# HpWang-whu/RoReg

Hardware: AMD Instinct MI355X
Metric: pair-registrations/sec (higher is better)
Workload: dtype f32 (every f32 operand enters the fp16 matrix cores as hi + lo fp16 under a per-keypoint power-of-two block scale: <= 22 significant bits relative to a CONSERVATIVE per-keypoint bound -- measured on the extractor: the bound sits 2^2..2^6 above the keypoint's true coefficient maximum (config.f16x2_sc

## Files before the change

include/roreg_hip.h:

```cpp
#ifndef ROREG_HIP_H
#define ROREG_HIP_H

#include <stdint.h>
#include <stddef.h>

#ifdef __cplusplus
extern "C" {
#endif

#define ROREG_ABI_VERSION 6
int roreg_abi_version(void);
const char *roreg_last_error(void);

int roreg_set_group_tables(const int32_t *P_host, const int32_t *Nei_host, const double *R_host);

size_t roreg_group_conv_packed_size(int Cin, int Cout, int KS);
int roreg_group_conv_pack_weights(const float *W_host , int Cin, int Cout, int KS,
                                  float *wpack_host );
size_t roreg_group_conv_workspace_size(int B, int Cin, int Cout, int Lin, int Lout, int KS);
int roreg_group_conv(const float *x, const float *wpack, const float *bias,
                     const float *bn_scale, const float *bn_shift, const float *residual,
                     float *out, const int32_t *gather,
                     int B, int Cin, int Cout, int Lin, int Lout, int KS,
                     float *workspace, size_t workspace_floats, void *stream);
// ... 175 lines not shown

int roreg_knn_attention(const float *qp, const float *kp, const float *vp, const int64_t *idx, int k_is_table, int v_is_table,
                        int m, int k, float *x_out, void *stream);

int roreg_rm_elementwise(int op, const float *a, const float *b, const float *c, const int64_t *idx, int L, int k, int C,
                         float *out, float *ws, void *stream);

size_t roreg_sinkhorn_workspace_size(int m, int n);
int roreg_sinkhorn(const float *src_final, int m, const float *tgt_final, int n, float alpha, int iters, float *Z_out,
                   int64_t *matches0, int64_t *matches1, float *mscores0, float *mscores1, float *ws, size_t ws_floats, void *stream);

size_t roreg_sinkhorn_batch_workspace_size(int n_seg, int max_m, int max_n, long long total_m, long long total_n);
int roreg_sinkhorn_batch_consts(const int32_t *seg_src_host, const int32_t *seg_tgt_host, int n_seg, float *consts_host);
int roreg_sinkhorn_batch(const float *src_final, const float *tgt_final, const int32_t *seg_src, const int32_t *seg_tgt,
                         const int32_t *seg_src_host, const int32_t *seg_tgt_host, const float *consts, int n_seg, float alpha, int iters,
                         int64_t *matches0, int64_t *matches1, float *mscores0, float *mscores1, float *ws, size_t ws_floats,
                         void *stream);

size_t roreg_sinkhorn_batch2_workspace_size(int n_seg, int max_m, int max_n, long long total_m, long long total_n);
int roreg_sinkhorn_batch2(const float *src_final, const float *tgt_final, const int32_t *seg_src, const int32_t *seg_tgt,
                          const int32_t *seg_src_host, const int32_t *seg_tgt_host, const float *consts, int n_seg, float alpha, int iters,
                          int64_t *matches0, int64_t *matches1, float *mscores0, float *mscores1, float *ws, size_t ws_floats,
                          int recompute, void *stream);
size_t roreg_sinkhorn_batch3_workspace_size(int n_seg, int max_m, int max_n, long long total_m, long long total_n, int recompute, int want_Z);
int roreg_sinkhorn_batch3(const float *src_final, const float *tgt_final, const int32_t *seg_src, const int32_t *seg_tgt,
                          const int32_t *seg_src_host, const int32_t *seg_tgt_host, const float *consts, int n_seg, float alpha, int iters,
                          int64_t *matches0, int64_t *matches1, float *mscores0, float *mscores1, float *ws, size_t ws_floats,
                          int recompute, float *Z_out, void *stream);
int roreg_write_files(const char *const *paths, const void *const *headers, const int32_t *header_len, const void *const *data,
                      const int64_t *nbytes, int n, int n_threads);
int roreg_yohoc_draw_many(const uint32_t *seeds, int n_pairs, const int64_t *anchors, const int64_t *offsets, int max_iter, int max_tries,
                          int64_t *rows_out, int32_t *n_hyp_out, double *giveup_out, int n_threads);
size_t roreg_mlp_head_workspace(int L, int n_seg, int C1);
int roreg_mlp_head(const float *x, const float *pos, const float *table, const int64_t *idx, const float *conf, int m, int k, int L, int Cin,
                   const float *W1, const float *b1, int C1, const float *Wr, const float *br, float *h, float *y, const int32_t *seg_off,
                   int n_seg, int mult, float eps, float *mean_rstd, double *ws, void *stream);
int roreg_sinkhorn_early_exit(int on);
int roreg_sinkhorn_iteration_stats(long long *iterations, long long *pairs, int reset, void *stream);

int roreg_set_fourier_tables(const float *F_host);
size_t roreg_irrep_gemm_tiles(int O, int B, int32_t *tiles_host);
size_t roreg_irrep_gemm_tiles_m(int O, int B, int tile_m , int32_t *tiles_host);
int roreg_irrep_gemm(const float *const *X, float *const *Out, const float *const *Add, const float *const *Wpack, int C, int O, int B,
                     const int32_t *tiles_dev, int n_tiles, void *stream);
int roreg_irrep_gemm_split(const float *const *X, float *const *Out, const float *const *Add, const void *const *Wsplit, int C, int O, int B,
                           const int32_t *tiles_dev, int n_tiles, void *stream);
int roreg_irrep_gemm_f16x2(const float *const *X, float *const *Out, const float *const *Add, const void *const *Wsplit2,
                           const float *x_bound_dev, int w_exp, const float *next_u_dev, const float *next_v_dev, float *out_bound_dev,
                           int C, int O, int B, const int32_t *tiles_dev, int n_tiles,
                           int tile_m ,
                           int x_planes , void *stream);
int roreg_gemm_persistent(int on);
int roreg_gemm_thin(int on);
int roreg_row_bound(const void *x_spatial, int x_bf16 , const float *bn_scale, const float *bn_shift,
                    float *bound_out, int B, int C, void *stream);
int roreg_ft_nonlin(const float *Xin , const float *x_spatial, const float *bias,
                    const float *bias2, const float *bn_scale, const float *bn_shift, const float *resid_spatial,
                    float *Xout , float *out_spatial ,
                    const int32_t *g_map ,
                    int Lout , int Lvalid,
                    int B, int C, int split ,
                    const float *out_bound ,
                    float *out_rowmax ,
                    int spatial_bf16 ,
                    int out_planes ,
                    void *stream);
int roreg_ft_nonlin_packed(const float *Xin, const float *bias, const float *bn_scale, const float *bn_shift, uint32_t *out_words,
                           const int32_t *g_map, int Lout, int Lvalid, int B, int C, const float *out_bound, float *raw_col, int raw_g,
                           void *stream);
int roreg_ft_nonlin_gathered(const uint64_t *rows , const int64_t *dr , int feat_bf16, const float *bn_scale ,
                             const float *bn_shift, float *Xout, int B, const float *out_bound , int out_planes, void *stream);

typedef struct roreg_icp_grid_desc {
    double origin[3];
    double edge;
    int32_t dims[3];
    int32_t n;
    int64_t cells;
    int64_t reserved;
} roreg_icp_grid_desc;
size_t roreg_icp_grid_size(const double *lo_host, const double *hi_host, int n, double max_dist, roreg_icp_grid_desc *desc_host,
                           size_t *workspace_bytes);
int roreg_icp_grid_build(const float *points, const roreg_icp_grid_desc *desc_host, void *grid, void *workspace, size_t workspace_bytes,
                         void *stream);
typedef struct roreg_icp_task {
    const void *tgt_grid;
    const void *src_grid;
    const double *T0;
    int32_t n_src;
    int32_t slot0;
} roreg_icp_task;
size_t roreg_icp_batch_workspace(int n_tasks, long long total_slots);
int roreg_icp_batch(const roreg_icp_task *tasks, int n_tasks, const int32_t *work, int n_work, long long total_slots, double max_dist,
                    int max_iter, double tol_deg, double tol_t, double *T_out, int32_t *iters_out, int32_t *inliers_out, double *rmse_out,
                    int32_t *status_out, int32_t *assign_out, double *stats_out, void *workspace, size_t workspace_bytes, void *stream);

int roreg_icp_normals(const void *grid, double radius, int min_neighbors, double *out, void *stream);
typedef struct roreg_icp_plane_task {
    const void *tgt_grid;
    const void *src_grid;
    const double *tgt_normals;
    const double *T0;
    int32_t n_src;
    int32_t slot0;
} roreg_icp_plane_task;
size_t roreg_icp_plane_batch_workspace(int n_tasks, long long total_slots);
// ... 49 lines not shown
```

roreg_amd/_abi.py:

```python
import ctypes
from ctypes import c_int, c_void_p, c_size_t, c_double, c_float, c_char_p

import numpy as np

ABI_VERSION = 6

_P = c_void_p
PROTOTYPES = {
    'roreg_abi_version': (c_int, []),
    'roreg_last_error': (c_char_p, []),
    'roreg_set_group_tables': (c_int, [_P, _P, _P]),
    'roreg_group_conv_packed_size': (c_size_t, [c_int, c_int, c_int]),
    'roreg_group_conv_pack_weights': (c_int, [_P, c_int, c_int, c_int, _P]),
    'roreg_group_conv_workspace_size': (c_size_t, [c_int, c_int, c_int, c_int, c_int, c_int]),
    'roreg_group_conv': (c_int, [_P, _P, _P, _P, _P, _P, _P, _P, c_int, c_int, c_int, c_int, c_int, c_int, _P, c_size_t, _P]),
    'roreg_group_conv_split': (c_int, [_P, _P, _P, _P, _P, _P, _P, _P, c_int, c_int, c_int, c_int, c_int, c_int, c_int, _P]),
    'roreg_group_conv_f16x2': (c_int, [_P, _P, c_int, _P, _P, _P, c_float, c_float, _P, _P, _P, _P, _P, c_int, c_int, c_int, c_int, c_int, c_int, c_int, _P]),
    'roreg_group_conv_f16x2_packed': (c_int, [_P, _P, c_int, _P, _P, _P, _P, _P, _P, c_int, c_int, c_int, c_int, c_int, c_int, c_int, _P]),
    'roreg_dense_f16x2': (c_int, [_P, _P, c_int, _P, _P, _P, c_float, c_float, _P, _P, c_int, _P, _P, c_int, c_int, c_int, _P]),
    'roreg_dense_split': (c_int, [_P, _P, _P, _P, _P, _P, c_int, _P, c_int, c_int, c_int, _P]),
    'roreg_gf_finalize': (c_int, [_P, _P, c_int, _P, c_int, _P]),
    'roreg_det_score': (c_int, [_P, _P, c_int, _P]),
    'roreg_inv_descriptor': (c_int, [_P, c_int, _P, c_int, _P]),
    'roreg_nn_search': (c_int, [_P, _P, c_int, _P, _P, c_int, c_int, _P, _P, _P, _P]),
# ... 3 lines not shown
    'roreg_knn_search': (c_int, [_P, c_int, _P, c_int, c_int, c_int, _P, _P, c_size_t, _P]),
    'roreg_knn_search_ex': (c_int, [_P, c_int, _P, c_int, c_int, c_int, c_int, _P, _P, _P, c_size_t, _P]),
    'roreg_knn_search_seg_workspace': (c_size_t, [ctypes.c_longlong, c_int, c_int, c_int]),
    'roreg_knn_search_seg': (c_int, [_P, _P, _P, _P, c_int, ctypes.c_longlong, c_int, c_int, c_int, c_int, _P, _P, c_size_t, _P]),
    'roreg_mutual_matches': (c_int, [_P, _P, c_int, c_int, _P, _P, _P, _P, _P]),
    'roreg_mutual_match_batch_workspace': (c_size_t, [c_int, c_int]),
    'roreg_mutual_match_batch': (c_int, [_P, c_int, c_int, _P, _P, _P, c_size_t, _P]),
    'roreg_des2r': (c_int, [_P, _P, _P, _P, c_int, _P, _P, _P]),
    'roreg_set_des2r_tables': (c_int, [c_int, _P, _P, _P, _P]),
    'roreg_group_corr_irrep': (c_int, [_P, _P, _P, _P, c_int, c_int, _P, _P]),
    'roreg_group_corr_mfma': (c_int, [_P, _P, _P, _P, c_int, c_int, _P, _P]),
    'roreg_des2r_irrep': (c_int, [_P, _P, _P, _P, _P, _P, c_int, c_int, _P, _P]),
    'roreg_des2r_recheck_count': (c_int, [c_int, _P]),
    'roreg_feat_coefs': (c_int, [_P, c_int, _P, c_int, c_int, c_int, _P]),
    'roreg_et_gather': (c_int, [_P, _P, _P, _P, c_int, _P, _P, _P, c_int, _P, _P]),
    'roreg_quat_to_trans': (c_int, [_P, _P, _P, _P, _P, _P, c_int, _P, _P, _P]),
    'roreg_ransac_score': (c_int, [_P, _P, _P, c_int, c_int, _P, _P, c_int, c_double, _P, _P, _P, _P]),
    'roreg_refine': (c_int, [_P, _P, _P, c_int, c_int, _P, c_int, _P, _P, _P, c_double, _P, _P, _P]),
    'roreg_lt_prepare_batch': (c_int, [_P, c_int, c_int, c_int, _P, _P, _P, _P, _P, _P]),
    'roreg_lt_finish_batch': (c_int, [_P, c_int, c_int, _P, _P, _P, _P]),
    'roreg_role_max': (c_int, [_P, _P, c_int, _P, _P, _P, c_int, _P]),
    'roreg_row_bound_roles': (c_int, [_P, c_int, _P, _P, _P, _P, c_int, _P]),
    'roreg_inv_descriptor_roles': (c_int, [_P, c_int, _P, _P, _P, _P, c_int, _P]),
    'roreg_lt_prepare_rows': (c_int, [_P, _P, c_int, c_int, c_int, _P, _P, _P, _P]),
    'roreg_ransac_batch_workspace': (c_size_t, [c_int, ctypes.c_longlong, c_int]),
    'roreg_ransac_batch': (c_int, [_P, c_int, ctypes.c_longlong, c_int, c_int, c_double, c_int, _P, _P, _P, _P, _P, _P, c_size_t, _P]),
    'roreg_refine_batch': (c_int, [_P, _P, c_int, ctypes.c_longlong, _P, ctypes.c_double, c_int, _P, _P, _P, _P]),
    'roreg_yohoc_draw': (c_int, [_P, ctypes.c_longlong, _P, _P, c_int, c_int, _P, _P, _P, _P]),
    'roreg_gather_rows_batch': (c_int, [_P, c_int, c_int, c_int, _P]),
    'roreg_gather_rows_f64': (c_int, [_P, _P, c_int, c_int, _P, _P]),
    'roreg_group_corr': (c_int, [_P, _P, _P, _P, c_int, c_int, _P, _P, _P]),
    'roreg_topk_dot_workspace_size': (c_size_t, [c_int, c_int, c_int]),
    'roreg_topk_dot': (c_int, [_P, c_int, _P, c_int, c_int, _P, _P, _P, c_size_t, _P, _P, c_int, c_int, c_int, _P]),
    'roreg_context_colmax': (c_int, [_P, c_int, _P, c_int, c_int, _P, _P, _P]),
    'roreg_sinkhorn_batch_workspace_size': (c_size_t, [c_int, c_int, c_int, ctypes.c_longlong, ctypes.c_longlong]),
    'roreg_sinkhorn_batch_consts': (c_int, [_P, _P, c_int, _P]),
    'roreg_sinkhorn_batch': (c_int, [_P, _P, _P, _P, _P, _P, _P, c_int, c_float, c_int, _P, _P, _P, _P, _P, c_size_t, _P]),
    'roreg_sinkhorn_batch2_workspace_size': (c_size_t, [c_int, c_int, c_int, ctypes.c_longlong, ctypes.c_longlong]),
    'roreg_sinkhorn_batch2': (c_int, [_P, _P, _P, _P, _P, _P, _P, c_int, c_float, c_int, _P, _P, _P, _P, _P, c_size_t, c_int, _P]),
    'roreg_sinkhorn_batch3_workspace_size': (c_size_t, [c_int, c_int, c_int, ctypes.c_longlong, ctypes.c_longlong, c_int, c_int]),
    'roreg_sinkhorn_batch3': (c_int, [_P, _P, _P, _P, _P, _P, _P, c_int, c_float, c_int, _P, _P, _P, _P, _P, c_size_t, c_int, _P, _P]),
    'roreg_write_files': (c_int, [_P, _P, _P, _P, _P, c_int, c_int]),
    'roreg_yohoc_draw_many': (c_int, [_P, c_int, _P, _P, c_int, c_int, _P, _P, _P, c_int]),
    'roreg_mlp_head_workspace': (c_size_t, [c_int, c_int, c_int]),
    'roreg_mlp_head': (c_int, [_P, _P, _P, _P, _P, c_int, c_int, c_int, c_int, _P, _P, c_int, _P, _P, _P, _P, _P, c_int, c_int, c_float, _P, _P, _P]),
    'roreg_sinkhorn_early_exit': (c_int, [c_int]),
    'roreg_sinkhorn_iteration_stats': (c_int, [_P, _P, c_int, _P]),
    'roreg_linear': (c_int, [_P, c_int, c_int, _P, _P, c_int, _P, _P]),
    'roreg_linear_mfma': (c_int, [_P, c_int, c_int, _P, _P, c_int, _P, _P]),
    'roreg_linear_path': (c_int, [c_int]),
    'roreg_linear_cat3': (c_int, [_P, _P, _P, _P, c_int, c_int, _P, _P, c_int, _P, _P]),
    'roreg_gemm_persistent': (c_int, [c_int]),
    'roreg_gemm_thin': (c_int, [c_int]),
    'roreg_instnorm_stats': (c_int, [_P, c_int, c_int, c_float, _P, _P, _P, c_int, c_int, _P]),
    'roreg_mlp_tail': (c_int, [_P, c_int, c_int, _P, _P, _P, _P, _P, c_int, c_int, _P]),
    'roreg_mlp_tail_mfma': (c_int, [_P, c_int, c_int, _P, _P, _P, _P, _P, c_int, c_int, _P]),
    'roreg_knn_attention': (c_int, [_P, _P, _P, _P, c_int, c_int, c_int, c_int, _P, _P]),
    'roreg_rm_elementwise': (c_int, [c_int, _P, _P, _P, _P, c_int, c_int, c_int, _P, _P, _P]),
    'roreg_sinkhorn_workspace_size': (c_size_t, [c_int, c_int]),
    'roreg_sinkhorn': (c_int, [_P, c_int, _P, c_int, c_float, c_int, _P, _P, _P, _P, _P, _P, c_size_t, _P]),
    'roreg_icp_grid_size': (c_size_t, [_P, _P, c_int, c_double, _P, _P]),
    'roreg_icp_grid_build': (c_int, [_P, _P, _P, _P, c_size_t, _P]),
    'roreg_icp_batch_workspace': (c_size_t, [c_int, ctypes.c_longlong]),
    'roreg_icp_batch': (c_int, [_P, c_int, _P, c_int, ctypes.c_longlong, c_double, c_int, c_double, c_double, _P, _P, _P, _P, _P, _P, _P, _P, c_size_t, _P]),
    'roreg_icp_normals': (c_int, [_P, c_double, c_int, _P, _P]),
    'roreg_icp_plane_batch_workspace': (c_size_t, [c_int, ctypes.c_longlong]),
    'roreg_icp_plane_batch': (c_int, [_P, c_int, _P, c_int, ctypes.c_longlong, c_double, c_int, c_double, c_double, _P, _P, _P, _P, _P, _P, _P, _P, c_size_t, _P]),
    'roreg_icp_gicp_batch_workspace': (c_size_t, [c_int, ctypes.c_longlong]),
    'roreg_icp_gicp_batch': (c_int, [_P, c_int, _P, c_int, ctypes.c_longlong, c_double, c_int, c_double, c_double, _P, _P, _P, _P, _P, _P, _P, _P, c_size_t, _P]),
    'roreg_icp_eval_workspace': (c_size_t, [c_int, ctypes.c_longlong]),
    'roreg_icp_eval_batch': (c_int, [_P, c_int, _P, c_int, ctypes.c_longlong, c_double, _P, _P, _P, _P, _P, c_size_t, _P]),
    'roreg_voxel_workspace': (c_size_t, [c_int]),
    'roreg_voxel_downsample': (c_int, [_P, c_int, c_double, _P, _P, _P, _P, _P, _P, _P, c_size_t, _P]),
    'roreg_pg_workspace': (c_size_t, [_P, c_int]),
    'roreg_pg_optimize_batch': (c_int, [_P, _P, c_int, _P, _P, _P, _P, _P, _P, _P, _P, _P, _P, _P, c_int, c_int, _P, _P, _P, _P, _P, _P, _P, _P, _P, _P, _P, c_size_t, _P]),
    'roreg_profile_enable': (c_int, [c_int]),
    'roreg_profile_read': (c_int, [c_int, _P, _P]),
    'roreg_set_fourier_tables': (c_int, [_P]),
    'roreg_mt_shuffle_prefix': (c_int, [_P, c_int, _P, c_int, c_int, _P, c_int]),
    'roreg_mt_stream_shuffle_prefix': (c_int, [_P, _P, _P, c_int, c_int, _P]),
    'roreg_irrep_gemm_tiles': (c_size_t, [c_int, c_int, _P]),
    'roreg_irrep_gemm_tiles_m': (c_size_t, [c_int, c_int, c_int, _P]),
    'roreg_irrep_gemm': (c_int, [_P, _P, _P, _P, c_int, c_int, c_int, _P, c_int, _P]),
    'roreg_irrep_gemm_split': (c_int, [_P, _P, _P, _P, c_int, c_int, c_int, _P, c_int, _P]),
    'roreg_irrep_gemm_f16x2': (c_int, [_P, _P, _P, _P, _P, c_int, _P, _P, _P, c_int, c_int, c_int, _P, c_int, c_int, c_int, _P]),
    'roreg_row_bound': (c_int, [_P, c_int, _P, _P, _P, c_int, c_int, _P]),
    'roreg_ft_nonlin': (c_int, [_P, _P, _P, _P, _P, _P, _P, _P, _P, _P, c_int, c_int, c_int, c_int, c_int, _P, _P, c_int, c_int, _P]),
    'roreg_ft_nonlin_packed': (c_int, [_P, _P, _P, _P, _P, _P, c_int, c_int, c_int, c_int, _P, _P, c_int, _P]),
    'roreg_ft_nonlin_gathered': (c_int, [_P, _P, c_int, _P, _P, _P, c_int, _P, c_int, _P]),
}


_RANSAC_TASK = np.dtype([('keys0', np.uint64), ('keys1', np.uint64), ('matches', np.uint64), ('w', np.uint64), ('Trans', np.uint64),
                         ('hyp_rows', np.uint64), ('M', np.int32), ('H', np.int32), ('koff', np.int64)])

_MATCH_TASK = np.dtype([('desc0', np.uint64), ('desc1', np.uint64), ('rows0', np.uint64), ('rows1', np.uint64), ('m0', np.int32), ('m1', np.int32)])

_GATHER_TASK = np.dtype([('src', np.uint64), ('rows', np.uint64), ('dst', np.uint64), ('n', np.int32), ('pad', np.int32)])

_LT_TASK = np.dtype([('before0', np.uint64), ('before1', np.uint64), ('after0', np.uint64), ('after1', np.uint64), ('keys0', np.uint64),
                     ('keys1', np.uint64), ('matches', np.uint64), ('sel', np.uint64), ('n', np.int32), ('pad', np.int32), ('off', np.int64),
                     ('coef0', np.uint64), ('coef1', np.uint64)])

_ICP_GRID_DESC = np.dtype([('origin', np.float64, 3), ('edge', np.float64), ('dims', np.int32, 3), ('n', np.int32), ('cells', np.int64),
                           ('reserved', np.int64)])

# ... 12 lines not shown
```

roreg_amd/csrc/mfma_match.hip:

```cpp
#include "common.h"
#include "primitives.h"

#pragma clang fp contract(off)

namespace {

struct MatchTask {
    const float *desc0, *desc1;
    const int64_t *rows0, *rows1;
    int32_t m0, m1;
};

constexpr int F = 32, TILE = 128, LP = 36;
constexpr float PAD_NORM = 1e30f;

struct WS {
    float *G;
    float *N;
    unsigned *AM;
    unsigned long long *PK;
    unsigned *MX;
};
__host__ __device__ inline size_t ws_task_bytes(int P) { return (size_t)2 * P * (F * 4 + 4 + 4 + 8) + 64; }
__device__ __forceinline__ WS ws_of(char *base, int task, int P) {
    char *p = base + (size_t)task * ws_task_bytes(P);
    WS w;
    w.PK = reinterpret_cast<unsigned long long *>(p); p += (size_t)2 * P * 8;
    w.G = reinterpret_cast<float *>(p); p += (size_t)2 * P * F * 4;
    w.N = reinterpret_cast<float *>(p); p += (size_t)2 * P * 4;
    w.AM = reinterpret_cast<unsigned *>(p); p += (size_t)2 * P * 4;
    w.MX = reinterpret_cast<unsigned *>(p);
    return w;
}

__device__ __forceinline__ unsigned f2o(float x) { const unsigned b = __float_as_uint(x); return b ^ ((b >> 31) ? 0xffffffffu : 0x80000000u); }
__device__ __forceinline__ float o2f(unsigned k) { return __uint_as_float(k ^ ((k >> 31) ? 0x80000000u : 0xffffffffu)); }

__global__ __launch_bounds__(256) void mm_prepare_kernel(const MatchTask *__restrict__ tasks, int P, char *__restrict__ wsb) {
    const int task = blockIdx.z >> 1, side = blockIdx.z & 1;
    const MatchTask t = tasks[task];
    const WS w = ws_of(wsb, task, P);
    const float *desc = side ? t.desc1 : t.desc0;
    const int64_t *rows = side ? t.rows1 : t.rows0;
    const int m = side ? t.m1 : t.m0;
    const int j = blockIdx.x * 8 + (threadIdx.x >> 5), f = threadIdx.x & 31;
    if (blockIdx.x == 0 && threadIdx.x == 0) w.MX[side] = 0u;
    if (j >= P) return;
    float v = 0.f;
    if (j < m) v = desc[(size_t)(rows ? rows[j] : (int64_t)j) * F + f];
    w.G[((size_t)side * P + j) * F + f] = v;
    float s = v * v;
#pragma unroll
    for (int o = 16; o > 0; o >>= 1) s += __shfl_xor(s, o);
    if (f == 0) {
// ... 120 lines not shown
#pragma unroll
        for (int b = 0; b < 2; ++b) {
            const int ic = wm * 64 + b * 32 + jl;
            const float ni = n0s[ic];
            float mn = __builtin_inff();
#pragma unroll
            for (int a = 0; a < 2; ++a)
#pragma unroll
                for (int r = 0; r < 16; ++r) {
                    const int jr = cd_row32(r, h, wn * 64 + a * 32);
                    mn = fminf(mn, (ni + n1s[jr]) - 2.f * DOT_CT(a, b, r, jr, ic));
                }
            mn = fminf(mn, __shfl_xor(mn, 32));
            if (h == 0 && i0 + ic < t.m0) atomicMin(&w.AM[i0 + ic], f2o(mn));
        }
    } else {
#pragma unroll
        for (int b = 0; b < 2; ++b) {
            const int jc = wn * 64 + b * 32 + jl;
            const float nj = n1s[jc], tj = thr1[jc];
#pragma unroll
            for (int a = 0; a < 2; ++a)
#pragma unroll
                for (int r = 0; r < 16; ++r) {
                    const int ir = cd_row32(r, h, wm * 64 + a * 32);
                    const float av = (n0s[ir] + nj) - 2.f * DOT_C(a, b, r, ir, jc);
                    const bool k0 = av <= thr0[ir], k1 = av <= tj;
                    if (k0 || k1) {
                        const float d = exact_dist(S + ir * LP, T + jc * LP);
                        const unsigned long long db = (unsigned long long)__float_as_uint(d) << 32;
                        if (k0 && j0 + jc < t.m1) atomicMin(&w.PK[i0 + ir], db | (unsigned)(j0 + jc));
                        if (k1 && i0 + ir < t.m0) atomicMin(&w.PK[(size_t)P + j0 + jc], db | (unsigned)(i0 + ir));
                    }
                }
        }
    }
#undef DOT_C
#undef DOT_CT
}

constexpr int TP = TILE * F;
__device__ __forceinline__ int swz_piece(int row, int c) { return row * 8 + (c ^ ((row >> 1) & 7)); }
__device__ __forceinline__ float exact_dist_swz(const float *__restrict__ s_tile, int ir, const float *__restrict__ t_tile, int jc) {
    float acc = 0.f;
#pragma unroll
    for (int f = 0; f < F; ++f) {
        const float sv = s_tile[swz_piece(ir, f >> 2) * 4 + (f & 3)], tv = t_tile[swz_piece(jc, f >> 2) * 4 + (f & 3)];
        const float d = __fsub_rn(sv, tv);
        acc = __fadd_rn(acc, __fmul_rn(d, d));
    }
    return sqrtf(__fadd_rn(acc, 1e-7f));
}

template <bool VERIFY>
__global__ __launch_bounds__(256, 2) void mm_strip_kernel(const MatchTask *__restrict__ tasks, int P, char *__restrict__ wsb) {
    extern __shared__ __attribute__((aligned(16))) char smem[];
    float *S = reinterpret_cast<float *>(smem);
    float *Tb = S + TP;
    float *n0s = Tb + 2 * TP, *xs0 = n0s + TILE, *is0 = xs0 + TILE, *thr0 = is0 + TILE;
    float *n1s = thr0 + TILE, *xs1 = n1s + 2 * TILE, *is1 = xs1 + 2 * TILE, *thr1 = is1 + 2 * TILE;
    unsigned *cm = reinterpret_cast<unsigned *>(thr1 + 2 * TILE);
    const int task = blockIdx.y;
    const MatchTask t = tasks[task];
    const int i0 = blockIdx.x * TILE;
    if (i0 >= t.m0 || t.m1 <= 0) return;
    const WS w = ws_of(wsb, task, P);
    const int tid = threadIdx.x, lane = tid & 63, wv = tid >> 6;
    const int wm = wv & 1, wn = wv >> 1, jl = lane & 31, h = lane >> 5;
    const int ntj = (t.m1 + TILE - 1) / TILE;
    const float mx0 = VERIFY ? __uint_as_float(w.MX[0]) : 0.f, mx1 = VERIFY ? __uint_as_float(w.MX[1]) : 0.f;

    auto dma_tile = [&](const float *src, float *dst) {
#pragma unroll
        for (int k = 0; k < 4; ++k) {
            const int q = k * 256 + tid, row = q >> 3, cs = q & 7;
            __builtin_amdgcn_global_load_lds((const __attribute__((address_space(1))) void *)(src + swz_piece(row, cs) * 4),
                                             (__attribute__((address_space(3))) void *)(dst + (k * 256 + wv * 64) * 4), 16, 0, 0);
        }
    };
    auto load_consts = [&](int jt) -> float {
        const int r = tid & (TILE - 1);
        if (tid < TILE) return w.N[(size_t)P + jt * TILE + r];
        return VERIFY ? o2f(w.AM[(size_t)P + jt * TILE + r]) : 0.f;
    };
    auto store_consts = [&](int buf, float v) {
        const int r = tid & (TILE - 1);
        if (tid < TILE) {
            const int e = norm_exp(v);
            n1s[buf * TILE + r] = v; xs1[buf * TILE + r] = ldexpf(1.f, e); is1[buf * TILE + r] = ldexpf(1.f, -e);
        } else if (VERIFY) thr1[buf * TILE + r] = v;
    };

    dma_tile(w.G + (size_t)i0 * F, S);
    dma_tile(w.G + (size_t)P * F, Tb);
    {
        const float c0 = load_consts(0);
        if (tid < TILE) {
            const float a = w.N[i0 + tid];
            const int e = norm_exp(a);
            n0s[tid] = a; xs0[tid] = ldexpf(1.f, e); is0[tid] = ldexpf(1.f, -e);
            if (VERIFY) thr0[tid] = o2f(w.AM[i0 + tid]) + (1e-4f * (a + mx1) + 1e-6f);
        }
        store_consts(0, c0);
        if (!VERIFY)
            for (int j = tid; j < P; j += 256) cm[j] = 0xffffffffu;
    }
    asm volatile("s_waitcnt vmcnt(0) lgkmcnt(0)" ::: "memory");
    __syncthreads();

    f16x8 sf[2][2][2];
#pragma unroll
    for (int st = 0; st < 2; ++st)
#pragma unroll
        for (int g = 0; g < 2; ++g) {
            const int rs = wm * 64 + g * 32 + jl;
            const float4 u0 = *reinterpret_cast<const float4 *>(S + swz_piece(rs, st * 4 + h * 2) * 4);
            const float4 u1 = *reinterpret_cast<const float4 *>(S + swz_piece(rs, st * 4 + h * 2 + 1) * 4);
            const float x8[8] = {u0.x, u0.y, u0.z, u0.w, u1.x, u1.y, u1.z, u1.w};
            split2(x8, xs0[rs], sf[st][g][0], sf[st][g][1]);
        }
    f32x16 rmin[2];
#pragma unroll
    for (int a = 0; a < 2; ++a)
#pragma unroll
        for (int r = 0; r < 16; ++r) rmin[a][r] = __builtin_inff();

    for (int jt = 0; jt < ntj; ++jt) {
        const int buf = jt & 1, j0 = jt * TILE;
        const float *T = Tb + buf * TP;
        float cnext = 0.f;
        if (jt + 1 < ntj) {
            dma_tile(w.G + ((size_t)P + j0 + TILE) * F, Tb + (buf ^ 1) * TP);
            cnext = load_consts(jt + 1);
        }
        f32x16 c[2][2];
#pragma unroll
        for (int a = 0; a < 2; ++a)
#pragma unroll
            for (int b = 0; b < 2; ++b)
#pragma unroll
                for (int r = 0; r < 16; ++r) c[a][b][r] = 0.f;
#pragma unroll
        for (int st = 0; st < 2; ++st) {
            f16x8 tf[2][2];
#pragma unroll
            for (int g = 0; g < 2; ++g) {
                const int rt = wn * 64 + g * 32 + jl;
                const float4 v0 = *reinterpret_cast<const float4 *>(T + swz_piece(rt, st * 4 + h * 2) * 4);
                const float4 v1 = *reinterpret_cast<const float4 *>(T + swz_piece(rt, st * 4 + h * 2 + 1) * 4);
                const float x8[8] = {v0.x, v0.y, v0.z, v0.w, v1.x, v1.y, v1.z, v1.w};
                split2(x8, xs1[buf * TILE + rt], tf[g][0], tf[g][1]);
            }
#pragma unroll
            for (int a = 0; a < 2; ++a)
#pragma unroll
                for (int b = 0; b < 2; ++b) c[a][b] = split_mma<2>(sf[st][a], tf[b], c[a][b]);
        }
#pragma unroll
        for (int b = 0; b < 2; ++b) {
            const int jc = wn * 64 + b * 32 + jl;
            const float nj = n1s[buf * TILE + jc], isj = is1[buf * TILE + jc];
            if constexpr (!VERIFY) {
                float mn = __builtin_inff();
#pragma unroll
                for (int a = 0; a < 2; ++a)
#pragma unroll
                    for (int r = 0; r < 16; ++r) {
                        const int ir = cd_row32(r, h, wm * 64 + a * 32);
                        const float av = (n0s[ir] + nj) - 2.f * ((c[a][b][r] * is0[ir]) * isj);
                        mn = fminf(mn, av);
                        rmin[a][r] = fminf(rmin[a][r], av);
                    }
                mn = fminf(mn, __shfl_xor(mn, 32));
                if (h == 0) atomicMin(cm + j0 + jc, f2o(mn));
            } else {
                const float tj = thr1[buf * TILE + jc] + (1e-4f * (nj + mx0) + 1e-6f);
                unsigned m0 = 0u, m1 = 0u;
#pragma unroll
                for (int a = 0; a < 2; ++a)
#pragma unroll
                    for (int r = 0; r < 16; ++r) {
                        const int ir = cd_row32(r, h, wm * 64 + a * 32);
                        const float av = (n0s[ir] + nj) - 2.f * ((c[a][b][r] * is0[ir]) * isj);
                        m0 |= (av <= thr0[ir] ? 1u : 0u) << (a * 16 + r);
                        m1 |= (av <= tj ? 1u : 0u) << (a * 16 + r);
                    }
                unsigned m = m0 | m1;
                while (m) {
                    const int q = __ffs(m) - 1;
                    m &= m - 1;
                    const int ir = cd_row32(q & 15, h, wm * 64 + (q >> 4) * 32);
                    const float d = exact_dist_swz(S, ir, T, jc);
                    const unsigned long long db = (unsigned long long)__float_as_uint(d) << 32;
                    if (((m0 >> q) & 1u) && j0 + jc < t.m1) atomicMin(&w.PK[i0 + ir], db | (unsigned)(j0 + jc));
                    if (((m1 >> q) & 1u) && i0 + ir < t.m0) atomicMin(&w.PK[(size_t)P + j0 + jc], db | (unsigned)(i0 + ir));
                }
            }
        }
        if (jt + 1 < ntj) store_consts(buf ^ 1, cnext);
        asm volatile("s_waitcnt vmcnt(0) lgkmcnt(0)" ::: "memory");
        __syncthreads();
    }
    if constexpr (!VERIFY) {
#pragma unroll
        for (int a = 0; a < 2; ++a)
#pragma unroll
            for (int r = 0; r < 16; ++r) {
                float v = rmin[a][r];
#pragma unroll
                for (int o = 16; o > 0; o >>= 1) v = fminf(v, __shfl_xor(v, o));
                const int ir = cd_row32(r, h, wm * 64 + a * 32);
                if (jl == 0 && i0 + ir < t.m0) atomicMin(&w.AM[i0 + ir], f2o(v));
            }
        for (int j = tid; j < t.m1; j += 256) atomicMin(&w.AM[(size_t)P + j], cm[j]);
    }
}

__global__ __launch_bounds__(1024) void mm_mutual_kernel(const MatchTask *__restrict__ tasks, int P, char *__restrict__ wsb, int out_pitch,
                                                         int64_t *__restrict__ match_all, int32_t *__restrict__ counts) {
    __shared__ int wave_cnt[16];
    __shared__ int base;
    const int task = blockIdx.x;
    const MatchTask t = tasks[task];
    const WS w = ws_of(wsb, task, P);
    const unsigned long long *p01 = w.PK, *p10 = w.PK + P;
    int64_t *match_out = match_all + (size_t)task * out_pitch * 2;
    const int m = t.m1 > 0 ? t.m0 : 0;
    const int tid = threadIdx.x, lane = tid & 63, wv = tid >> 6;
    if (tid == 0) base = 0;
    __syncthreads();
    for (int start = 0; start < m; start += 1024) {
        const int i = start + tid;
        bool keep = false;
        int64_t j = 0;
        if (i < m) {
            j = (int64_t)(p01[i] & 0xffffffffu);
            keep = j < (int64_t)t.m1 && (int64_t)(p10[j] & 0xffffffffu) == (int64_t)i;
        }
        const unsigned long long mask = __ballot(keep);
        const int before = __popcll(mask & ((1ull << lane) - 1ull));
        if (lane == 0) wave_cnt[wv] = __popcll(mask);
        __syncthreads();
        int woff = 0, total = 0;
#pragma unroll
        for (int q = 0; q < 16; ++q) {
            const int cq = wave_cnt[q];
            if (q < wv) woff += cq;
            total += cq;
        }
        const int b0 = base;
        if (keep) {
            const int pos = b0 + woff + before;
            match_out[2 * pos] = t.rows0 ? t.rows0[i] : (int64_t)i;
            match_out[2 * pos + 1] = t.rows1 ? t.rows1[j] : j;
        }
        __syncthreads();
        if (tid == 0) base = b0 + total;
        __syncthreads();
    }
    if (tid == 0) counts[task] = base;
}

}

extern "C" size_t roreg_mutual_match_batch_workspace(int n_tasks, int max_m) {
    const int P = (max_m + TILE - 1) / TILE * TILE;
    return (size_t)n_tasks * ws_task_bytes(P > 0 ? P : TILE);
}

extern "C" int roreg_mutual_match_batch(const roreg_match_task *tasks_dev, int n_tasks, int max_m, int64_t *match_out, int32_t *counts_out,
                                        void *workspace, size_t workspace_bytes, void *stream) {
    if (n_tasks == 0) return 0;
    ROREG_REQUIRE(tasks_dev && match_out && counts_out && workspace && n_tasks > 0 && max_m >= 0, "roreg_mutual_match_batch: bad arguments");
    ROREG_REQUIRE(workspace_bytes >= roreg_mutual_match_batch_workspace(n_tasks, max_m), "roreg_mutual_match_batch: workspace too small");
    ROREG_REQUIRE(n_tasks <= 65535, "roreg_mutual_match_batch: too many tasks in one call (%d)", n_tasks);
    static_assert(sizeof(roreg_match_task) == sizeof(MatchTask), "roreg_match_task layout");
    hipStream_t s = roreg::as_stream(stream);
    const MatchTask *tasks = reinterpret_cast<const MatchTask *>(tasks_dev);
    const int P = max_m > 0 ? (max_m + TILE - 1) / TILE * TILE : TILE;
    char *ws = reinterpret_cast<char *>(workspace);
    const int out_pitch = (max_m + 1) & ~1;
    if (max_m > 0) {
        hipLaunchKernelGGL(mm_prepare_kernel, dim3(P / 8, 1, 2 * n_tasks), dim3(256), 0, s, tasks, P, ws);
        hipLaunchKernelGGL(mm_maxnorm_kernel, dim3(P / 256 + 1, 1, 2 * n_tasks), dim3(256), 0, s, tasks, P, ws);
        const dim3 grid(P / TILE, P / TILE, n_tasks);
        roreg::ProfScope prof(roreg::PROF_MM_TILE, s);
        static const bool bf16x3 = [] { const char *e = getenv("ROREG_MATCH_BF16X3"); return e && e[0] == '1'; }();
        static const bool tiles = [] { const char *e = getenv("ROREG_MATCH_TILES"); return e && e[0] == '1'; }();
        const size_t lds_strip = (size_t)(3 * TP + 12 * TILE) * 4 + (size_t)P * 4;
        if (!bf16x3 && !tiles && lds_strip <= 80 * 1024) {
            const dim3 sgrid(P / TILE, n_tasks);
            if (roreg::launch_lds("roreg_mutual_match_batch", mm_strip_kernel<false>, sgrid, dim3(256), lds_strip, s, tasks, P, ws) ||
                roreg::launch_lds("roreg_mutual_match_batch", mm_strip_kernel<true>, sgrid, dim3(256), lds_strip, s, tasks, P, ws)) return 1;
        } else if (bf16x3) {
            hipLaunchKernelGGL((mm_tile_kernel<false, 3>), grid, dim3(256), 0, s, tasks, P, ws);
            hipLaunchKernelGGL((mm_tile_kernel<true, 3>), grid, dim3(256), 0, s, tasks, P, ws);
        } else {
            hipLaunchKernelGGL((mm_tile_kernel<false, 2>), grid, dim3(256), 0, s, tasks, P, ws);
            hipLaunchKernelGGL((mm_tile_kernel<true, 2>), grid, dim3(256), 0, s, tasks, P, ws);
        }
    }
    hipLaunchKernelGGL(mm_mutual_kernel, dim3(n_tasks), dim3(1024), 0, s, tasks, P, ws, out_pitch, match_out, counts_out);
    ROREG_CHECK_LAUNCH("roreg_mutual_match_batch");
    return 0;
}
```

roreg_amd/hip.py:

```python
import ctypes
import os
import threading
from ctypes import c_int, c_void_p, c_size_t, c_double, c_float, c_char_p

import numpy as np
import torch

from .group import tables

_LIB_PATH = os.environ.get('ROREG_HIP_LIB') or os.path.join(os.path.dirname(os.path.abspath(__file__)), 'libroreg_hip.so')

GEMM_MODES = ('f16x2', 'bf16x3', 'f32')
GEMM_MODE = os.environ.get('ROREG_GEMM', 'f16x2')
if GEMM_MODE == 'split':
    GEMM_MODE = 'bf16x3'
if GEMM_MODE not in GEMM_MODES:
    raise ValueError(f"ROREG_GEMM must be one of {GEMM_MODES}, got {GEMM_MODE!r}")
XDMA = os.environ.get('ROREG_GEMM_XDMA', '1') == '1'
MFMA16 = os.environ.get('ROREG_GEMM_MFMA16', '1') == '1'


def use_planes(O):
    return bool(XDMA and O % 256 == 0 and not os.environ.get('ROREG_TILE_M128'))
_lib = None
# ... 645 lines not shown
    ws_n = lib().roreg_ransac_batch_workspace(n, koff, max_H)
    ws = torch.empty(max(ws_n, 8) // 8, dtype=torch.float64, device=dev)
    _check(lib().roreg_ransac_batch(_ptr(tdev), n, koff, max(max_M, 1), max_H, float(ird), int(bool(w_f32)), _ptr(best), _ptr(T1), _ptr(st1), _ptr(T2), _ptr(st2),
                                    _ptr(ws), ws_n, _stream()), 'roreg_ransac_batch')
    if keep:
        return best, T1, st1, T2, st2, (tdev, ws, koff, bool(w_f32), tasks)
    return best, T1, st1, T2, st2


def refine_batch(ctx, sel, T_in, dist):
    tdev, ws, total_M, w_f32, _tasks = ctx
    n = len(sel)
    dev = ws.device
    T = torch.empty((n, 4, 4), dtype=torch.float64, device=dev); st = torch.empty((n, 16), dtype=torch.float64, device=dev)
    if n == 0:
        return T, st
    sel_dev = upload(np.ascontiguousarray(sel, np.int32))
    Tin = T_in if torch.is_tensor(T_in) else upload(np.ascontiguousarray(T_in, np.float64))
    _check(lib().roreg_refine_batch(_ptr(tdev), _ptr(sel_dev, torch.int32), n, total_M, _ptr(Tin, torch.float64), float(dist), int(w_f32), _ptr(T), _ptr(st),
                                    _ptr(ws), _stream()), 'roreg_refine_batch')
    return T, st




def mutual_match_batch(tasks):
    n = len(tasks)
    table = np.zeros(n, _MATCH_TASK)
    keep = []
    for i, (d0, d1, r0, r1) in enumerate(tasks):
        if d0.shape[1] != 32 or d1.shape[1] != 32:
            raise HipError('mutual_match_batch: descriptors must be [*,32] float32')
        for t in (d0, d1):
            _ptr(t, torch.float32)
        table[i] = (d0.data_ptr(), d1.data_ptr(), r0.data_ptr() if r0 is not None else 0, r1.data_ptr() if r1 is not None else 0,
                    r0.shape[0] if r0 is not None else d0.shape[0], r1.shape[0] if r1 is not None else d1.shape[0])
        for t in (r0, r1):
            if t is not None:
                _ptr(t, torch.int64)
    dev = tasks[0][0].device if n else torch.device('cuda')
    max_m = int(max([0] + [max(int(t['m0']), int(t['m1'])) for t in table]))
    pitch = (max_m + 1) & ~1
    out = torch.empty((n, max(pitch, 1), 2), dtype=torch.int64, device=dev)
    cnt = torch.zeros(max(n, 1), dtype=torch.int32, device=dev)[:n]
    if n == 0:
        return out, cnt
    tdev = upload(table.view(np.uint8).reshape(n, _MATCH_TASK.itemsize))
    ws_n = lib().roreg_mutual_match_batch_workspace(n, max_m)
    ws = torch.empty(max(ws_n, 8) // 8, dtype=torch.int64, device=dev)
    _check(lib().roreg_mutual_match_batch(_ptr(tdev), n, max_m, _ptr(out), _ptr(cnt), _ptr(ws), ws_n, _stream()), 'roreg_mutual_match_batch')
    return out, cnt


_des2r_ready = False


def des2r_tables(transpose=False):
    from .fourier import group_fourier, DIMS
    gf = group_fourier(); T = tables()
    ia = np.zeros((60, 5), np.uint8); ib = np.zeros((60, 5), np.uint8); cnt = np.zeros(60, np.uint8)
    NT = np.zeros((60, 60), np.float64)
    for q, (ri, i, j) in enumerate(gf.index):
        d = DIMS[ri]; off = int(gf.offsets[ri])
        cnt[q] = d
        for k in range(5):
            kk = min(k, d - 1)
            if not transpose:
                ia[q, k] = off + i * d + kk; ib[q, k] = off + j * d + kk
            else:
                ia[q, k] = off + kk * d + j; ib[q, k] = off + kk * d + i
        NT[q, :] = gf.rho[ri][:, j, i]
    rng = np.random.default_rng(0)
    d1 = rng.standard_normal((4, 60)); d2 = rng.standard_normal((4, 60))
    perm = (lambda a: T.P[:, a]) if transpose else (lambda a: T.P[a])
    want = np.array([(d1[:, perm(a)] * d2).sum() for a in range(60)])
    X1 = d1 @ gf.F.T; X2 = d2 @ gf.F.T
    C = np.array([sum((X2[f, ia[q, :cnt[q]]] * X1[f, ib[q, :cnt[q]]]).sum() for f in range(4)) for q in range(60)])
    assert np.abs(C @ NT - want).max() < 1e-11, 'irrep-domain correlation identity violated'
    return ia, ib, cnt, np.ascontiguousarray(NT, np.float32)


def ensure_des2r():
    global _des2r_ready
    if not _des2r_ready:
        ensure_tables(); ensure_fourier()
        for mode in (0, 1):
            ia, ib, cnt, NT = des2r_tables(transpose=bool(mode))
            _check(lib().roreg_set_des2r_tables(mode, ia.ctypes.data, ib.ctypes.data, cnt.ctypes.data, NT.ctypes.data), 'roreg_set_des2r_tables')
        _des2r_ready = True


def feat_coefs(x):
    ensure_fourier()
    B, C = int(x.shape[0]), int(x.shape[1])
    out = torch.empty((B, C, 60), dtype=torch.float32, device=x.device)
    xp, bf = _feat(x)
    _check(lib().roreg_feat_coefs(xp, bf, _ptr(out), B, C, {'f16x2': 2, 'bf16x3': 1, 'f32': 0}[GEMM_MODE], _stream()), 'roreg_feat_coefs')
    return out


def des2r_recheck_count(reset=True):
    ensure_des2r()
    n = ctypes.c_int32(0)
    _check(lib().roreg_des2r_recheck_count(1 if reset else 0, ctypes.byref(n)), 'roreg_des2r_recheck_count')
    return n.value

# ... 149 lines not shown
```

Before: 1114.

## Add uniform-scale mutual-match strip kernel folding norms into the MFMA

Adds a specialized mutual-match strip kernel that runs when both point sets' max norms have close power-of-two exponents. It scales the features by fixed exponents and folds the squared-norm terms into an extra fp16 MFMA step, so the distance comes straight out of the accumulator. The row and column extremes then reduce with med3-based max instead of separate distance arithmetic. Tasks that fail the uniform check fall back to a guarded copy of the original kernel, which doubles the launches per pass and adds scaling-precision risk.

```diff
diff --git a/include/roreg_hip.h b/include/roreg_hip.h
--- a/include/roreg_hip.h
+++ b/include/roreg_hip.h
@@ -251,6 +251,7 @@
                            int x_planes , void *stream);
 int roreg_gemm_persistent(int on);
 int roreg_gemm_thin(int on);
+int roreg_match_uniform(int on);
 int roreg_row_bound(const void *x_spatial, int x_bf16 , const float *bn_scale, const float *bn_shift,
                     float *bound_out, int B, int C, void *stream);
 int roreg_ft_nonlin(const float *Xin , const float *x_spatial, const float *bias,
diff --git a/roreg_amd/_abi.py b/roreg_amd/_abi.py
--- a/roreg_amd/_abi.py
+++ b/roreg_amd/_abi.py
@@ -79,6 +79,7 @@
     'roreg_linear_cat3': (c_int, [_P, _P, _P, _P, c_int, c_int, _P, _P, c_int, _P, _P]),
     'roreg_gemm_persistent': (c_int, [c_int]),
     'roreg_gemm_thin': (c_int, [c_int]),
+    'roreg_match_uniform': (c_int, [c_int]),
     'roreg_instnorm_stats': (c_int, [_P, c_int, c_int, c_float, _P, _P, _P, c_int, c_int, _P]),
     'roreg_mlp_tail': (c_int, [_P, c_int, c_int, _P, _P, _P, _P, _P, c_int, c_int, _P]),
     'roreg_mlp_tail_mfma': (c_int, [_P, c_int, c_int, _P, _P, _P, _P, _P, c_int, c_int, _P]),
diff --git a/roreg_amd/csrc/mfma_match.hip b/roreg_amd/csrc/mfma_match.hip
--- a/roreg_amd/csrc/mfma_match.hip
+++ b/roreg_amd/csrc/mfma_match.hip
@@ -1,5 +1,7 @@
 #include "common.h"
 #include "primitives.h"
+#include <atomic>
+#include <stdlib.h>
 
 #pragma clang fp contract(off)
 
@@ -226,7 +228,25 @@
     return sqrtf(__fadd_rn(acc, 1e-7f));
 }
 
-template <bool VERIFY>
+__device__ __forceinline__ void dma_tile_swz(const float *src, float *dst, int tid, int wv) {
+#pragma unroll
+    for (int k = 0; k < 4; ++k) {
+        const int q = k * 256 + tid, row = q >> 3, cs = q & 7;
+        __builtin_amdgcn_global_load_lds((const __attribute__((address_space(1))) void *)(src + swz_piece(row, cs) * 4),
+                                         (__attribute__((address_space(3))) void *)(dst + (k * 256 + wv * 64) * 4), 16, 0, 0);
+    }
+}
+
+constexpr int U_DMAX = 3, U_EMAX = 24;
+__device__ __forceinline__ bool uniform_form(const unsigned *__restrict__ MX, int &e0, int &e1) {
+    const float mx0 = __uint_as_float(MX[0]), mx1 = __uint_as_float(MX[1]);
+    e0 = norm_exp(mx0); e1 = norm_exp(mx1);
+    const int d = e1 - e0;
+    return mx0 > 0.f && mx1 > 0.f && mx0 < __builtin_inff() && mx1 < __builtin_inff() && d >= -U_DMAX && d <= U_DMAX &&
+           e0 <= U_EMAX && e1 <= U_EMAX;
+}
+
+template <bool VERIFY, bool GUARDED = false>
 __global__ __launch_bounds__(256, 2) void mm_strip_kernel(const MatchTask *__restrict__ tasks, int P, char *__restrict__ wsb) {
     extern __shared__ __attribute__((aligned(16))) char smem[];
     float *S = reinterpret_cast<float *>(smem);
@@ -239,19 +259,15 @@
     const int i0 = blockIdx.x * TILE;
     if (i0 >= t.m0 || t.m1 <= 0) return;
     const WS w = ws_of(wsb, task, P);
+    if constexpr (GUARDED) {
+        int e0, e1;
+        if (uniform_form(w.MX, e0, e1)) return;
+    }
     const int tid = threadIdx.x, lane = tid & 63, wv = tid >> 6;
     const int wm = wv & 1, wn = wv >> 1, jl = lane & 31, h = lane >> 5;
     const int ntj = (t.m1 + TILE - 1) / TILE;
     const float mx0 = VERIFY ? __uint_as_float(w.MX[0]) : 0.f, mx1 = VERIFY ? __uint_as_float(w.MX[1]) : 0.f;
 
-    auto dma_tile = [&](const float *src, float *dst) {
-#pragma unroll
-        for (int k = 0; k < 4; ++k) {
-            const int q = k * 256 + tid, row = q >> 3, cs = q & 7;
-            __builtin_amdgcn_global_load_lds((const __attribute__((address_space(1))) void *)(src + swz_piece(row, cs) * 4),
-                                             (__attribute__((address_space(3))) void *)(dst + (k * 256 + wv * 64) * 4), 16, 0, 0);
-        }
-    };
     auto load_consts = [&](int jt) -> float {
         const int r = tid & (TILE - 1);
         if (tid < TILE) return w.N[(size_t)P + jt * TILE + r];
@@ -265,8 +281,8 @@
         } else if (VERIFY) thr1[buf * TILE + r] = v;
     };
 
-    dma_tile(w.G + (size_t)i0 * F, S);
-    dma_tile(w.G + (size_t)P * F, Tb);
+    dma_tile_swz(w.G + (size_t)i0 * F, S, tid, wv);
+    dma_tile_swz(w.G + (size_t)P * F, Tb, tid, wv);
     {
         const float c0 = load_consts(0);
         if (tid < TILE) {
@@ -304,7 +320,7 @@
         const float *T = Tb + buf * TP;
         float cnext = 0.f;
         if (jt + 1 < ntj) {
-            dma_tile(w.G + ((size_t)P + j0 + TILE) * F, Tb + (buf ^ 1) * TP);
+            dma_tile_swz(w.G + ((size_t)P + j0 + TILE) * F, Tb + (buf ^ 1) * TP, tid, wv);
             cnext = load_consts(jt + 1);
         }
         f32x16 c[2][2];
@@ -385,6 +401,172 @@
                 for (int o = 16; o > 0; o >>= 1) v = fminf(v, __shfl_xor(v, o));
                 const int ir = cd_row32(r, h, wm * 64 + a * 32);
                 if (jl == 0 && i0 + ir < t.m0) atomicMin(&w.AM[i0 + ir], f2o(v));
+            }
+        for (int j = tid; j < t.m1; j += 256) atomicMin(&w.AM[(size_t)P + j], cm[j]);
+    }
+}
+
+__device__ __forceinline__ float opaque_inf() { float x; asm("s_mov_b32 %0, 0x7f800000" : "=s"(x)); return x; }
+__device__ __forceinline__ float max_med3(float a, float b, float pinf) { return __builtin_amdgcn_fmed3f(a, b, pinf); }
+template <bool S_SIDE>
+__device__ __forceinline__ f16x8 norm_step_frag(float n, bool pad, float vscale , float k_mine , int h) {
+    const float v = pad ? 0.f : n * vscale;
+    const _Float16 hi = (_Float16)v, lo = (_Float16)(v - (float)hi), kc = (_Float16)k_mine, z = (_Float16)0.f;
+    const _Float16 big = (_Float16)32768.f, pd = pad ? (_Float16)-65504.f : z;
+    f16x8 f;
+    if (S_SIDE) {
+        if (h == 0) { f[0] = -hi; f[1] = -lo; f[2] = kc; f[3] = kc; f[4] = pd; f[5] = pd; f[6] = pd; f[7] = pd; }
+        else { f[0] = big; f[1] = big; f[2] = big; f[3] = big; f[4] = z; f[5] = z; f[6] = z; f[7] = z; }
+    } else {
+        if (h == 0) { f[0] = kc; f[1] = kc; f[2] = -hi; f[3] = -lo; f[4] = big; f[5] = big; f[6] = big; f[7] = big; }
+        else { f[0] = pd; f[1] = pd; f[2] = pd; f[3] = pd; f[4] = z; f[5] = z; f[6] = z; f[7] = z; }
+    }
+    return f;
+}
+
+template <bool VERIFY>
+__global__ __launch_bounds__(256, 2) void mm_strip_uniform_kernel(const MatchTask *__restrict__ tasks, int P, char *__restrict__ wsb) {
+    extern __shared__ __attribute__((aligned(16))) char smem[];
+    float *S = reinterpret_cast<float *>(smem);
+    float *Tb = S + TP;
+    float *n0s = Tb + 2 * TP, *thr0 = n0s + TILE;
+    float *n1s = thr0 + TILE, *am1 = n1s + 2 * TILE;
+    unsigned *cm = reinterpret_cast<unsigned *>(am1 + 2 * TILE);
+    const int task = blockIdx.y;
+    const MatchTask t = tasks[task];
+    const int i0 = blockIdx.x * TILE;
+    if (i0 >= t.m0 || t.m1 <= 0) return;
+    const WS w = ws_of(wsb, task, P);
+    int e0, e1;
+    if (!uniform_form(w.MX, e0, e1)) return;
+    const int tid = threadIdx.x, lane = tid & 63, wv = tid >> 6, jl = lane & 31, h = lane >> 5;
+    const int ntj = (t.m1 + TILE - 1) / TILE;
+    const float mx0 = __uint_as_float(w.MX[0]), mx1 = __uint_as_float(w.MX[1]);
+    const float xs0 = ldexpf(1.f, e0), xs1 = ldexpf(1.f, e1), vs0 = ldexpf(1.f, 2 * e0 - 13), vs1 = ldexpf(1.f, 2 * e1 - 13);
+    const float kS = ldexpf(1.f, 12 - (e1 - e0)), kT = ldexpf(1.f, 12 + (e1 - e0));
+    const float hsc = ldexpf(1.f, e0 + e1 - 1);
+    const float pinf = opaque_inf();
+
+    auto load_consts = [&](int jt) -> float {
+        const int r = tid & (TILE - 1);
+        if (tid < TILE) return w.N[(size_t)P + jt * TILE + r];
+        return VERIFY ? o2f(w.AM[(size_t)P + jt * TILE + r]) : 0.f;
+    };
+    auto store_consts = [&](int buf, float v) {
+        const int r = tid & (TILE - 1);
+        if (tid < TILE) n1s[buf * TILE + r] = v;
+        else if (VERIFY) am1[buf * TILE + r] = v;
+    };
+
+    dma_tile_swz(w.G + (size_t)i0 * F, S, tid, wv);
+    dma_tile_swz(w.G + (size_t)P * F, Tb, tid, wv);
+    {
+        const float c0 = load_consts(0);
+        if (tid < TILE) {
+            const float a = w.N[i0 + tid];
+            n0s[tid] = a;
+            if (VERIFY) thr0[tid] = -o2f(w.AM[i0 + tid]) - (1e-4f * (a + mx1) + 1e-6f) * hsc;
+        }
+        store_consts(0, c0);
+    }
+    asm volatile("s_waitcnt vmcnt(0) lgkmcnt(0)" ::: "memory");
+    __syncthreads();
+
+    f16x8 sf[2][4][2], sn[4];
+#pragma unroll
+    for (int g = 0; g < 4; ++g) {
+        const int rs = g * 32 + jl;
+#pragma unroll
+        for (int st = 0; st < 2; ++st) {
+            const float4 u0 = *reinterpret_cast<const float4 *>(S + swz_piece(rs, st * 4 + h * 2) * 4);
+            const float4 u1 = *reinterpret_cast<const float4 *>(S + swz_piece(rs, st * 4 + h * 2 + 1) * 4);
+            const float x8[8] = {u0.x, u0.y, u0.z, u0.w, u1.x, u1.y, u1.z, u1.w};
+            split2(x8, xs0, sf[st][g][0], sf[st][g][1]);
+        }
+        sn[g] = norm_step_frag<true>(n0s[rs], i0 + rs >= t.m0, vs0, kS, h);
+    }
+    f32x16 rmax[VERIFY ? 1 : 4];
+    if constexpr (!VERIFY) {
+#pragma unroll
+        for (int a = 0; a < 4; ++a)
+#pragma unroll
+            for (int r = 0; r < 16; ++r) rmax[a][r] = -__builtin_inff();
+    }
+
+    for (int jt = 0; jt < ntj; ++jt) {
+        const int buf = jt & 1, j0 = jt * TILE;
+        const float *T = Tb + buf * TP;
+        float cnext = 0.f;
+        if (jt + 1 < ntj) {
+            dma_tile_swz(w.G + ((size_t)P + j0 + TILE) * F, Tb + (buf ^ 1) * TP, tid, wv);
+            cnext = load_consts(jt + 1);
+        }
+        const int jc = wv * 32 + jl;
+        const float nj = n1s[buf * TILE + jc];
+        f16x8 tf[2][2];
+#pragma unroll
+        for (int st = 0; st < 2; ++st) {
+            const float4 v0 = *reinterpret_cast<const float4 *>(T + swz_piece(jc, st * 4 + h * 2) * 4);
+            const float4 v1 = *reinterpret_cast<const float4 *>(T + swz_piece(jc, st * 4 + h * 2 + 1) * 4);
+            const float x8[8] = {v0.x, v0.y, v0.z, v0.w, v1.x, v1.y, v1.z, v1.w};
+            split2(x8, xs1, tf[st][0], tf[st][1]);
+        }
+        const f16x8 tn = norm_step_frag<false>(nj, j0 + jc >= t.m1, vs1, kT, h);
+        float mn = -__builtin_inff();
+        float tj = 0.f;
+        if constexpr (VERIFY) tj = -am1[buf * TILE + jc] - (1e-4f * (nj + mx0) + 1e-6f) * hsc;
+#pragma unroll
+        for (int a = 0; a < 4; ++a) {
+            f32x16 c;
+#pragma unroll
+            for (int r = 0; r < 16; ++r) c[r] = 0.f;
+            c = split_mma<2>(sf[0][a], tf[0], c);
+            c = split_mma<2>(sf[1][a], tf[1], c);
+            c = mfma_32x32x16(sn[a], tn, c);
+            if constexpr (!VERIFY) {
+#pragma unroll
+                for (int r = 0; r < 16; ++r) {
+                    mn = max_med3(mn, c[r], pinf);
+                    rmax[a][r] = max_med3(rmax[a][r], c[r], pinf);
+                }
+            } else {
+                unsigned m0 = 0u, m1 = 0u;
+#pragma unroll
+                for (int r = 0; r < 16; ++r) {
+                    const int ir = cd_row32(r, h, a * 32);
+                    m0 |= (c[r] >= thr0[ir] ? 1u : 0u) << r;
+                    m1 |= (c[r] >= tj ? 1u : 0u) << r;
+                }
+                unsigned m = m0 | m1;
+                while (m) {
+                    const int q = __ffs(m) - 1;
+                    m &= m - 1;
+                    const int ir = cd_row32(q, h, a * 32);
+                    const float d = exact_dist_swz(S, ir, T, jc);
+                    const unsigned long long db = (unsigned long long)__float_as_uint(d) << 32;
+                    if (((m0 >> q) & 1u) && j0 + jc < t.m1) atomicMin(&w.PK[i0 + ir], db | (unsigned)(j0 + jc));
+                    if (((m1 >> q) & 1u) && i0 + ir < t.m0) atomicMin(&w.PK[(size_t)P + j0 + jc], db | (unsigned)(i0 + ir));
+                }
+            }
+        }
+        if constexpr (!VERIFY) {
+            mn = fmaxf(mn, __shfl_xor(mn, 32));
+            if (h == 0) cm[j0 + jc] = f2o(-mn);
+        }
+        if (jt + 1 < ntj) store_consts(buf ^ 1, cnext);
+        asm volatile("s_waitcnt vmcnt(0) lgkmcnt(0)" ::: "memory");
+        __syncthreads();
+    }
+    if constexpr (!VERIFY) {
+#pragma unroll
+        for (int a = 0; a < 4; ++a)
+#pragma unroll
+            for (int r = 0; r < 16; ++r) {
+                float v = rmax[a][r];
+#pragma unroll
+                for (int o = 16; o > 0; o >>= 1) v = fmaxf(v, __shfl_xor(v, o));
+                const int ir = cd_row32(r, h, a * 32);
+                if (jl == 0 && i0 + ir < t.m0) atomicMin(&w.AM[i0 + ir], f2o(-v));
             }
         for (int j = tid; j < t.m1; j += 256) atomicMin(&w.AM[(size_t)P + j], cm[j]);
     }
@@ -435,7 +617,21 @@
     if (tid == 0) counts[task] = base;
 }
 
-}
+int match_uniform_switch(int on) {
+    static std::atomic<int> v{-1};
+    int prev = v.load(std::memory_order_relaxed);
+    if (prev < 0) {
+        const char *e = getenv("ROREG_MATCH_UNIFORM");
+        prev = e && (e[0] == '0' || e[0] == '1') ? e[0] - '0' : 1;
+        v.store(prev, std::memory_order_relaxed);
+    }
+    if (on == 0 || on == 1) v.store(on, std::memory_order_relaxed);
+    return prev;
+}
+
+}
+
+extern "C" int roreg_match_uniform(int on) { return match_uniform_switch(on); }
 
 extern "C" size_t roreg_mutual_match_batch_workspace(int n_tasks, int max_m) {
     const int P = (max_m + TILE - 1) / TILE * TILE;
@@ -462,7 +658,13 @@
         static const bool bf16x3 = [] { const char *e = getenv("ROREG_MATCH_BF16X3"); return e && e[0] == '1'; }();
         static const bool tiles = [] { const char *e = getenv("ROREG_MATCH_TILES"); return e && e[0] == '1'; }();
         const size_t lds_strip = (size_t)(3 * TP + 12 * TILE) * 4 + (size_t)P * 4;
-        if (!bf16x3 && !tiles && lds_strip <= 80 * 1024) {
+        if (!bf16x3 && !tiles && lds_strip <= 80 * 1024 && match_uniform_switch(-1)) {
+            const dim3 sgrid(P / TILE, n_tasks);
+            if (roreg::launch_lds("roreg_mutual_match_batch", mm_strip_uniform_kernel<false>, sgrid, dim3(256), lds_strip, s, tasks, P, ws) ||
+                roreg::launch_lds("roreg_mutual_match_batch", mm_strip_kernel<false, true>, sgrid, dim3(256), lds_strip, s, tasks, P, ws) ||
+                roreg::launch_lds("roreg_mutual_match_batch", mm_strip_uniform_kernel<true>, sgrid, dim3(256), lds_strip, s, tasks, P, ws) ||
+                roreg::launch_lds("roreg_mutual_match_batch", mm_strip_kernel<true, true>, sgrid, dim3(256), lds_strip, s, tasks, P, ws)) return 1;
+        } else if (!bf16x3 && !tiles && lds_strip <= 80 * 1024) {
             const dim3 sgrid(P / TILE, n_tasks);
             if (roreg::launch_lds("roreg_mutual_match_batch", mm_strip_kernel<false>, sgrid, dim3(256), lds_strip, s, tasks, P, ws) ||
                 roreg::launch_lds("roreg_mutual_match_batch", mm_strip_kernel<true>, sgrid, dim3(256), lds_strip, s, tasks, P, ws)) return 1;
diff --git a/roreg_amd/hip.py b/roreg_amd/hip.py
--- a/roreg_amd/hip.py
+++ b/roreg_amd/hip.py
@@ -721,6 +721,10 @@
     return out, cnt
 
 
+def match_uniform(on=-1):
+    return int(lib().roreg_match_uniform(int(on)))
+
+
 _des2r_ready = False
 
 
```

After: 1120, median of 6. About the same (+0.6%).
